# qianduoduolr/FGVC

Hardware: AMD Instinct MI355X
Metric: frames/sec + ms/corr-volume, 480p 8-frame clip, 1/2/4/8 MI355X (higher is better)
Workload: dtype f16 + fp6 (e2m3) MFMA operands, f32 accumulate; top-k near-ties re-scored in f64 from f32 features

## Files before the change

### fgvc_amd/csrc/refine.hip

```cpp
#include "common.hpp"

namespace fgvc {

constexpr int RF_KX = 16;
constexpr int RF_KMAX = 10;
constexpr int RF_BRUTE = 1 << 30;

struct RefineItem {
  int row, q, flags, m;
  int gid[RF_KX];
  float sc[RF_KX];
};
static_assert(sizeof(RefineItem) == 144, "RefineItem");
constexpr int RF_INLINE = 1 << 29;
constexpr int RF_SAMPLE = 1 << 28;

struct RefineParams {
  const int32_t* pair_idx;
  const float* pair_score;
  const int32_t* slot_pair;
  const int4* pairs;
  const unsigned char* q_exact;
  const unsigned char* k_exact;
  long long q_frame_bytes, k_frame_bytes;
  int q_row_bytes, k_row_bytes;
  int T, Hq, Wq, Hk, Wk, kin, kout;
  float temperature, eps;
  int weight_mode;
  int r2max, ry, rx, reach_y, reach_x;
  int32_t* idx_out;
  float* logit_out;
  float* weight_out;
  int* counters;
  RefineItem* items;
  int* scan_ids;
  int* scan_done;
  unsigned long long* scan_parts;
  int scan_cap;
};

__device__ __forceinline__ void rf_write(const RefineParams& p, int row, int q, const float (&sc)[RF_KMAX], const int (&id)[RF_KMAX]) {
  float lg[RF_KMAX], w[RF_KMAX];
#pragma unroll
  for (int j = 0; j < RF_KMAX; ++j) lg[j] = sc[j] / p.temperature;
  if (p.weight_mode == FGVC_WEIGHT_SOFTMAX) {
    float sum = 0.f;
#pragma unroll
    for (int j = 0; j < RF_KMAX; ++j) {
      w[j] = (j < p.kout) ? expf(lg[j] - lg[0]) : 0.f;
      sum += w[j];
    }
#pragma unroll
    for (int j = 0; j < RF_KMAX; ++j) w[j] = w[j] / sum;
  } else {
#pragma unroll
    for (int j = 0; j < RF_KMAX; ++j) {
      const float c = fmaxf(lg[j], 0.f);
      w[j] = c * c;
    }
  }
  const size_t o = ((size_t)row * p.Hq * p.Wq + q) * p.kout;
#pragma unroll
  for (int j = 0; j < RF_KMAX; ++j) {
    if (j < p.kout) {
      p.idx_out[o + j] = id[j] == IDX_EMPTY ? -1 : id[j];
      p.logit_out[o + j] = lg[j];
      p.weight_out[o + j] = w[j];
    }
  }
}

__global__ __launch_bounds__(256) void merge_mark_kernel(RefineParams p) {
  const int HWq = p.Hq * p.Wq, HWk = p.Hk * p.Wk;
  const int q_raw = blockIdx.x * 256 + threadIdx.x;
  const int f = blockIdx.y;
  const bool valid = q_raw < HWq;
  const int q = valid ? q_raw : HWq - 1;
  TopK<RF_KX> top;
  top.init();
  float drop_max = -INFINITY;
  float tau_max = -INFINITY;
  float tau[16];
#pragma unroll
  for (int t = 0; t < 16; ++t) tau[t] = -INFINITY;
  auto take = [&](int t, int id, float s) -> bool {
    const int gid = t * HWk + id;
    if (!top.accepts(s, gid)) {
      drop_max = fmaxf(drop_max, s);
      return false;
    }
    if (top.ix[RF_KX - 1] != IDX_EMPTY) drop_max = fmaxf(drop_max, top.v[RF_KX - 1]);
    top.insert(s, gid);
    return true;
  };
  if (p.kin == RF_KMAX) {
    unsigned long long a[RF_KX];
#pragma unroll
    for (int j = 0; j < RF_KX; ++j) a[j] = 0ull;
    unsigned long long dropk = 0ull;
    int2 ii[RF_KMAX / 2], ni[RF_KMAX / 2];
    float2 ss[RF_KMAX / 2], ns[RF_KMAX / 2];
    auto fetch = [&](int t, int2 (&I)[RF_KMAX / 2], float2 (&S)[RF_KMAX / 2]) -> int {
      const int pid = t < p.T ? p.slot_pair[f * p.T + t] : -1;
      if (pid >= 0) {
        const size_t o = ((size_t)pid * HWq + q) * RF_KMAX;
#pragma unroll
        for (int j = 0; j < RF_KMAX / 2; ++j) {
          I[j] = reinterpret_cast<const int2*>(p.pair_idx + o)[j];
          S[j] = reinterpret_cast<const float2*>(p.pair_score + o)[j];
        }
      }
      return pid;
    };
    int pid = fetch(0, ii, ss);
    for (int t = 0; t < p.T; ++t) {
      const int npid = fetch(t + 1, ni, ns);
      if (pid >= 0) {
        unsigned long long bk[RF_KMAX];
#pragma unroll
        for (int j = 0; j < RF_KMAX; ++j) {
          const int id = (j & 1) ? ii[j / 2].y : ii[j / 2].x;
          const float sv = (j & 1) ? ss[j / 2].y : ss[j / 2].x;
          bk[j] = id >= 0 ? TopK64<1>::make_key(sv, t * HWk + id) : 0ull;
        }
        if (bk[RF_KMAX - 1] != 0ull) {
          const float tv = ss[RF_KMAX / 2 - 1].y;
          tau_max = fmaxf(tau_max, tv);
#pragma unroll
          for (int u = 0; u < 16; ++u) tau[u] = u == t ? tv : tau[u];
        }
#pragma unroll
        for (int i = RF_KX - RF_KMAX; i < RF_KX; ++i) {
          const unsigned long long x = a[i], y = bk[RF_KX - 1 - i];
          const bool g = x > y;
          a[i] = g ? x : y;
          const unsigned long long lo = g ? y : x;
          dropk = lo > dropk ? lo : dropk;
        }
#pragma unroll
        for (int d = RF_KX / 2; d >= 1; d >>= 1)
#pragma unroll
          for (int i = 0; i < RF_KX; ++i)
            if ((i & d) == 0) {
              const unsigned long long x = a[i], y = a[i + d];
              const bool g = x > y;
              a[i] = g ? x : y;
              a[i + d] = g ? y : x;
            }
      }
      pid = npid;
#pragma unroll
      for (int j = 0; j < RF_KMAX / 2; ++j) { ii[j] = ni[j]; ss[j] = ns[j]; }
    }
    TopK64<RF_KX> dec;
#pragma unroll
    for (int j = 0; j < RF_KX; ++j) dec.k[j] = a[j];
#pragma unroll
    for (int j = 0; j < RF_KX; ++j) {
      top.v[j] = dec.score(j);
      top.ix[j] = a[j] == 0ull ? IDX_EMPTY : dec.index(j);
    }
    if (dropk != 0ull) {
      TopK64<1> dd;
      dd.k[0] = dropk;
      drop_max = dd.score(0);
    }
  } else {
    for (int t = 0; t < p.T; ++t) {
      const int pid = p.slot_pair[f * p.T + t];
      if (pid < 0) continue;
      const size_t o = ((size_t)pid * HWq + q) * p.kin;
      if (p.pair_idx[o + p.kin - 1] >= 0) {
        const float tv = p.pair_score[o + p.kin - 1];
        tau_max = fmaxf(tau_max, tv);
#pragma unroll
        for (int u = 0; u < 16; ++u) tau[u] = u == t ? tv : tau[u];
      }
      for (int j = 0; j < p.kin; ++j) {
        const int id = p.pair_idx[o + j];
        if (id < 0) break;
        if (!take(t, id, p.pair_score[o + j])) break;
      }
    }
  }
  const float two_eps = 2.f * p.eps;
  float t_k = -INFINITY;
#pragma unroll
  for (int j = 0; j < RF_KX; ++j)
    if (j == p.kout - 1 && top.ix[j] != IDX_EMPTY) t_k = top.v[j];
  const float thr = t_k - two_eps;
  int m = 0;
#pragma unroll
  for (int j = 0; j < RF_KX; ++j) m += (top.ix[j] != IDX_EMPTY && top.v[j] >= thr) ? 1 : 0;
  const bool brute = (drop_max > -INFINITY && drop_max >= thr) || (tau_max > -INFINITY && tau_max >= thr);
  unsigned twins = 0;
#pragma unroll
  for (int j = 0; j + 1 < RF_KX; ++j) {
    if (j + 1 < m && top.v[j] == top.v[j + 1]) {
      const int ta = top.ix[j] / HWk, tb = top.ix[j + 1] / HWk;
      if (top.ix[j] - ta * HWk == top.ix[j + 1] - tb * HWk && p.slot_pair[f * p.T + ta] == p.slot_pair[f * p.T + tb]) twins |= 1u << j;
    }
  }
  unsigned mask = 0;
#pragma unroll
  for (int j = 0; j + 1 < RF_KX; ++j) {
    const bool inside = j + 1 < m;
    if (inside && !((twins >> j) & 1u) && top.v[j] - top.v[j + 1] <= two_eps) mask |= 3u << j;
  }
#pragma unroll
  for (int j = 0; j + 1 < RF_KX; ++j)
    if (((twins >> j) & 1u) && ((mask >> j) & 3u)) mask |= 3u << j;
#pragma unroll
  for (int j = RF_KX - 2; j >= 0; --j)
    if (((twins >> j) & 1u) && ((mask >> j) & 3u)) mask |= 3u << j;
  const bool flagged = valid && (brute || mask != 0u);
  if (valid && !flagged) {
    float sc[RF_KMAX];
    int id[RF_KMAX];
#pragma unroll
    for (int j = 0; j < RF_KMAX; ++j) { sc[j] = top.v[j]; id[j] = top.ix[j]; }
    rf_write(p, f, q, sc, id);
  }
  const unsigned hsh = ((unsigned)q * 2654435761u) ^ ((unsigned)f * 0x9E3779B1u);
  const bool sampled = valid && !flagged && ((hsh >> 11) & 63u) == 0u;
  unsigned mask_all = 0;
#pragma unroll
  for (int j = 0; j < RF_KX; ++j) mask_all |= (top.ix[j] != IDX_EMPTY) ? (1u << j) : 0u;
  const bool queued = flagged || (sampled && mask_all != 0u);
  const int lane = threadIdx.x & 63;
  const unsigned long long lt = (1ull << lane) - 1ull;
  const unsigned long long bf = __ballot(queued), bb = __ballot(flagged && brute);
  if (bf == 0ull) return;
  int base_f = 0, base_b = 0;
  if (lane == __builtin_ctzll(bf)) base_f = atomicAdd(&p.counters[0], __popcll(bf));
  base_f = __shfl(base_f, __builtin_ctzll(bf));
  if (bb != 0ull) {
    if (lane == __builtin_ctzll(bb)) base_b = atomicAdd(&p.counters[1], __popcll(bb));
    base_b = __shfl(base_b, __builtin_ctzll(bb));
  }
  int n_resc = (flagged && !brute) ? __popc(mask) : 0;
#pragma unroll
  for (int mm = 32; mm >= 1; mm >>= 1) n_resc += __shfl_xor(n_resc, mm);
  if (lane == __builtin_ctzll(bf) && n_resc) atomicAdd(&p.counters[2], n_resc);
  int n_smp = (queued && !flagged) ? __popc(mask_all) : 0;
#pragma unroll
  for (int mm = 32; mm >= 1; mm >>= 1) n_smp += __shfl_xor(n_smp, mm);
  const int q_smp = __popcll(__ballot(queued && !flagged));
  if (lane == __builtin_ctzll(bf) && n_smp) {
    atomicAdd(&p.counters[6], n_smp);
    atomicAdd(&p.counters[7], q_smp);
  }
  if (!queued) return;
  const int slot = base_f + __popcll(bf & lt);
  int flags = flagged ? (int)mask : (RF_SAMPLE | (int)mask_all);
  if (!flagged) m = __popc(mask_all);
  if (brute) {
    const int b = base_b + __popcll(bb & lt);
    unsigned open = 0;
#pragma unroll
    for (int t = 0; t < 16; ++t) open |= (tau[t] > -INFINITY && tau[t] >= thr) ? (1u << t) : 0u;
    if (drop_max > -INFINITY && drop_max >= thr) open = 0xffffu;
    flags = RF_BRUTE | (int)open;
    if (b < p.scan_cap) p.scan_ids[b] = slot;
    else { flags |= RF_INLINE; atomicAdd(&p.counters[3], 1); }
  }
  RefineItem* it = p.items + slot;
  it->row = f; it->q = q; it->flags = flags; it->m = m;
#pragma unroll
  for (int j = 0; j < RF_KX; ++j) { it->gid[j] = top.ix[j]; it->sc[j] = top.v[j]; }
}

__device__ __forceinline__ int rf_mine(int lane) { return ((lane >> 5) & 1) * 4 + ((lane >> 4) & 1) * 2 + ((lane >> 3) & 1); }
__device__ __forceinline__ void rf_load8(const unsigned char* const (&krow)[8], int lane, f32x4 (&b)[8]) {
#pragma unroll
  for (int v = 0; v < 8; ++v) b[v] = *reinterpret_cast<const f32x4*>(krow[v] + 16 * lane);
}
__device__ __forceinline__ double rf_reduce8(const f32x4& a, const f32x4 (&b)[8], int lane) {
  double p[8];
#pragma unroll
  for (int v = 0; v < 8; ++v) {
    double s = (double)a.x * (double)b[v].x;
    s = fma((double)a.y, (double)b[v].y, s);
    s = fma((double)a.z, (double)b[v].z, s);
    s = fma((double)a.w, (double)b[v].w, s);
    p[v] = s;
  }
  const bool h5 = (lane & 32) != 0, h4 = (lane & 16) != 0, h3 = (lane & 8) != 0;
  double q4[4], q2[2];
#pragma unroll
  for (int i = 0; i < 4; ++i) q4[i] = (h5 ? p[i + 4] : p[i]) + __shfl_xor(h5 ? p[i] : p[i + 4], 32);
#pragma unroll
  for (int i = 0; i < 2; ++i) q2[i] = (h4 ? q4[i + 2] : q4[i]) + __shfl_xor(h4 ? q4[i] : q4[i + 2], 16);
  double c = (h3 ? q2[1] : q2[0]) + __shfl_xor(h3 ? q2[0] : q2[1], 8);
  c += __shfl_xor(c, 4);
  c += __shfl_xor(c, 2);
  c += __shfl_xor(c, 1);
  return c;
}
__device__ __forceinline__ double rf_dot8(const f32x4& a, const unsigned char* const (&krow)[8], int lane) {
  f32x4 b[8];
  rf_load8(krow, lane, b);
  return rf_reduce8(a, b, lane);
}

__device__ __forceinline__ void refine_item_wave(const RefineParams& p, const RefineItem* I, int lane, float& wave_err) {
  const int HWk = p.Hk * p.Wk;
  {
    const int row = __builtin_amdgcn_readfirstlane(I->row), q = __builtin_amdgcn_readfirstlane(I->q);
    const int flags = __builtin_amdgcn_readfirstlane(I->flags);
    if ((flags & RF_BRUTE) && !(flags & RF_INLINE)) return;
    int m = __builtin_amdgcn_readfirstlane(I->m);
    int gid = I->gid[lane & 15];
    float sc = I->sc[lane & 15];
    int qf = 0;
    for (int t = 0; t < p.T; ++t) {
      const int pid = p.slot_pair[row * p.T + t];
      if (pid >= 0) { qf = p.pairs[pid].x; break; }
    }
    const f32x4 qv = *reinterpret_cast<const f32x4*>(p.q_exact + (size_t)qf * p.q_frame_bytes + (size_t)q * p.q_row_bytes + 16 * lane);
    if (!(flags & RF_BRUTE)) {
      float err = 0.f;
      const unsigned char* qrow = p.q_exact + (size_t)qf * p.q_frame_bytes + (size_t)q * p.q_row_bytes;
#pragma unroll
      for (int half = 0; half < 2; ++half) {
        if (!((flags >> (8 * half)) & 255)) continue;
        const unsigned char* kr[8];
#pragma unroll
        for (int v = 0; v < 8; ++v) {
          const int e = 8 * half + v;
          kr[v] = qrow;
          if ((flags >> e) & 1) {
            const int g = __builtin_amdgcn_readlane(gid, e);
            const int t = g / HWk, pix = g - t * HWk;
            const int kf = p.pairs[p.slot_pair[row * p.T + t]].y;
            kr[v] = p.k_exact + (size_t)kf * p.k_frame_bytes + (size_t)pix * p.k_row_bytes;
          }
        }
        const float sv = (float)rf_dot8(qv, kr, lane);
#pragma unroll
        for (int v = 0; v < 8; ++v) {
          const int e = 8 * half + v;
          const int src = ((v >> 2) & 1) * 32 + ((v >> 1) & 1) * 16 + (v & 1) * 8;
          const float got = __builtin_bit_cast(float, __builtin_amdgcn_readlane(__builtin_bit_cast(int, sv), src));
          if (((flags >> e) & 1) && (lane & 15) == e) {
            err = fmaxf(err, fabsf(got - sc));
            sc = got;
          }
        }
      }
      wave_err = fmaxf(wave_err, err);
    } else {
      TopK<RF_KMAX> ex;
      ex.init();
      const int qy = q / p.Wq, qx = q - qy * p.Wq;
      for (int t = 0; t < p.T; ++t) {
        const int pid = p.slot_pair[row * p.T + t];
        if (pid < 0) continue;
        const int4 pr = p.pairs[pid];
        const bool masked = (pr.z & FGVC_PAIR_MASKED) != 0;
        const int y0 = masked ? imax(0, qy - imin(p.reach_y, qy)) : 0, y1 = masked ? imin(p.Hk - 1, qy + imin(p.reach_y, p.Hk)) : p.Hk - 1;
        const int x0 = masked ? imax(0, qx - imin(p.reach_x, qx)) : 0, x1 = masked ? imin(p.Wk - 1, qx + imin(p.reach_x, p.Wk)) : p.Wk - 1;
        const unsigned char* kb = p.k_exact + (size_t)pr.y * p.k_frame_bytes;
        for (int y = y0; y <= y1; ++y)
          for (int x = x0; x <= x1; ++x) {
            if (masked) {
              const int dy = y - qy, dx = x - qx, ady = dy < 0 ? -dy : dy, adx = dx < 0 ? -dx : dx;
              const long long d2 = (long long)dy * dy + (long long)dx * dx;
              if (!(d2 <= p.r2max && ady <= p.ry && adx <= p.rx)) continue;
            }
            const int pix = y * p.Wk + x;
            const unsigned char* r1 = kb + (size_t)pix * p.k_row_bytes;
            const unsigned char* kr[8] = {r1, r1, r1, r1, r1, r1, r1, r1};
            const float s = (float)rf_dot8(qv, kr, lane);
            const int g = t * HWk + pix;
            if (ex.accepts(s, g)) ex.insert(s, g);
          }
      }
      gid = IDX_EMPTY; sc = -INFINITY; m = 0;
#pragma unroll
      for (int j = 0; j < RF_KMAX; ++j) {
        if ((lane & 15) == j) { gid = ex.ix[j]; sc = ex.v[j]; }
        m += ex.ix[j] != IDX_EMPTY ? 1 : 0;
      }
    }
    const int i = lane & 15;
    int rank = 0;
#pragma unroll
    for (int j = 0; j < RF_KX; ++j) {
      const float sj = __builtin_bit_cast(float, __builtin_amdgcn_readlane(__builtin_bit_cast(int, sc), j));
      const int gj = __builtin_amdgcn_readlane(gid, j);
      rank += (j < m && (sj > sc || (sj == sc && gj < gid))) ? 1 : 0;
    }
    float osc[RF_KMAX];
    int oid[RF_KMAX];
#pragma unroll
    for (int r = 0; r < RF_KMAX; ++r) {
      const unsigned long long b = __ballot(lane < 16 && i < m && rank == r);
      if (b) {
        const int src = __builtin_amdgcn_readfirstlane(__builtin_ctzll(b));
        osc[r] = __builtin_bit_cast(float, __builtin_amdgcn_readlane(__builtin_bit_cast(int, sc), src));
        oid[r] = __builtin_amdgcn_readlane(gid, src);
      } else {
        osc[r] = -INFINITY;
        oid[r] = IDX_EMPTY;
      }
    }
    if (lane == 0) rf_write(p, row, q, osc, oid);
  }
}


__global__ __launch_bounds__(256) void refine_kernel(RefineParams p) {
  const int lane = threadIdx.x & 63, sub = lane & 15, g0 = lane & 48;
  const int wave = __builtin_amdgcn_readfirstlane((int)((blockIdx.x * 256 + threadIdx.x) >> 6));
  const int n_waves = (int)gridDim.x * 4;
  const int n_items = __builtin_amdgcn_readfirstlane(p.counters[0]);
  const int HWk = p.Hk * p.Wk;
  float wave_err = 0.f, wave_err_s = 0.f;
  for (int base = 4 * wave; base < n_items; base += 4 * n_waves) {
    const int it = base + (lane >> 4);
    const bool active = it < n_items;
    const RefineItem* I = p.items + (active ? it : base);
    const int row = I->row, q = I->q, flags = I->flags, m = I->m;
    int gid = I->gid[sub];
    float sc = I->sc[sub];
    const bool mine = active && !(flags & RF_BRUTE);
    const unsigned mask = mine ? ((unsigned)flags & 0xffffu) : 0u;
    const bool ent = mine && gid != IDX_EMPTY && sub < m;
    const int t_ = ent ? gid / HWk : 0, pix = ent ? gid - t_ * HWk : 0;
    const int pid = ent ? p.slot_pair[row * p.T + t_] : -1;
    const int4 pr = pid >= 0 ? p.pairs[pid] : int4{0, 0, 0, 0};
    const unsigned char* my_row = p.k_exact + (size_t)pr.y * p.k_frame_bytes + (size_t)pix * p.k_row_bytes;
    const int qf = __shfl(pr.x, g0);
    const unsigned char* qrow = p.q_exact + (size_t)qf * p.q_frame_bytes + (size_t)(mine ? q : 0) * p.q_row_bytes + 64 * sub;
    f32x4 qv[4];
    if (mine) {
#pragma unroll
      for (int j = 0; j < 4; ++j) qv[j] = *reinterpret_cast<const f32x4*>(qrow + 16 * j);
    } else {
#pragma unroll
      for (int j = 0; j < 4; ++j) qv[j] = f32x4{0.f, 0.f, 0.f, 0.f};
    }
    float err = 0.f;
    unsigned um = mask;
    um |= __shfl_xor(um, 16);
    um |= __shfl_xor(um, 32);
    um = (unsigned)__builtin_amdgcn_readfirstlane((int)um);
    while (um) {
      int ev[4];
      bool nd[4];
      f32x4 kv[4][4];
#pragma unroll
      for (int b4 = 0; b4 < 4; ++b4) {
        ev[b4] = um ? __builtin_ctz(um) : -1;
        if (um) um &= um - 1;
        nd[b4] = ev[b4] >= 0 && ((mask >> ev[b4]) & 1u);
        const unsigned long long ra = __shfl((unsigned long long)(size_t)my_row, g0 + (ev[b4] >= 0 ? ev[b4] : 0));
        const unsigned char* kr = nd[b4] ? reinterpret_cast<const unsigned char*>((size_t)ra) + 64 * sub : qrow;
#pragma unroll
        for (int j = 0; j < 4; ++j) kv[b4][j] = *reinterpret_cast<const f32x4*>(kr + 16 * j);
      }
#pragma unroll
      for (int b4 = 0; b4 < 4; ++b4) {
        if (ev[b4] < 0) continue;
        double sacc = 0.0;
#pragma unroll
        for (int j = 0; j < 4; ++j) {
          sacc = fma((double)qv[j].x, (double)kv[b4][j].x, sacc);
          sacc = fma((double)qv[j].y, (double)kv[b4][j].y, sacc);
          sacc = fma((double)qv[j].z, (double)kv[b4][j].z, sacc);
          sacc = fma((double)qv[j].w, (double)kv[b4][j].w, sacc);
        }
#pragma unroll
        for (int mm = 8; mm >= 1; mm >>= 1) sacc += __shfl_xor(sacc, mm);
        if (nd[b4] && sub == ev[b4]) {
          const float got = (float)sacc;
          err = fmaxf(err, fabsf(got - sc));
          sc = got;
        }
      }
    }
    const bool smp = mine && (flags & RF_SAMPLE) != 0;
    wave_err_s = fmaxf(wave_err_s, smp ? err : 0.f);
    wave_err = fmaxf(wave_err, smp ? 0.f : err);
    int rank = 0;
#pragma unroll
    for (int j = 0; j < RF_KX; ++j) {
      const float sj = __shfl(sc, g0 + j);
      const int gj = __shfl(gid, g0 + j);
      rank += (j < m && (sj > sc || (sj == sc && gj < gid))) ? 1 : 0;
    }
    const bool inwin = mine && !smp && sub < m;
    float osc[RF_KMAX];
    int oid[RF_KMAX];
#pragma unroll
    for (int r = 0; r < RF_KMAX; ++r) {
      const unsigned long long bal = __ballot(inwin && rank == r);
      const unsigned grp = (unsigned)(bal >> g0) & 0xffffu;
      const int src = g0 + (grp ? __builtin_ctz(grp) : 0);
      const float v = __shfl(sc, src);
      const int gi = __shfl(gid, src);
      osc[r] = grp ? v : -INFINITY;
      oid[r] = grp ? gi : IDX_EMPTY;
    }
    if (mine && !smp && sub == 0) rf_write(p, row, q, osc, oid);
  }
#pragma unroll
  for (int mm = 32; mm >= 1; mm >>= 1) {
    wave_err = fmaxf(wave_err, __shfl_xor(wave_err, mm));
    wave_err_s = fmaxf(wave_err_s, __shfl_xor(wave_err_s, mm));
  }
  if (lane == 0 && wave_err > 0.f) atomicMax(&p.counters[4], __builtin_bit_cast(int, wave_err));
  if (lane == 0 && wave_err_s > 0.f) atomicMax(&p.counters[5], __builtin_bit_cast(int, wave_err_s));
}

__global__ __launch_bounds__(256) void refine_inline_kernel(RefineParams p) {
  if (p.counters[3] == 0) return;
  const int lane = threadIdx.x & 63;
  const int wave = __builtin_amdgcn_readfirstlane((int)((blockIdx.x * 256 + threadIdx.x) >> 6));
  const int n_waves = (int)gridDim.x * 4;
  const int n_items = __builtin_amdgcn_readfirstlane(p.counters[0]);
  float wave_err = 0.f;
  for (int it = wave; it < n_items; it += n_waves) {
    const int flags = __builtin_amdgcn_readfirstlane(p.items[it].flags);
    if ((flags & RF_BRUTE) && (flags & RF_INLINE)) refine_item_wave(p, p.items + it, lane, wave_err);
  }
}

constexpr int RF_SCAN_WAVES = 8;
constexpr int RF_SCAN_PARTS = 4;

__global__ __launch_bounds__(RF_SCAN_WAVES * 64) void refine_scan_kernel(RefineParams p) {
  __shared__ unsigned long long wk[RF_SCAN_WAVES][8 * RF_KMAX];
  __shared__ unsigned long long wl[RF_SCAN_WAVES][RF_KMAX];
  __shared__ unsigned long long pl[RF_KMAX];
  __shared__ unsigned long long fk[RF_SCAN_PARTS * RF_KMAX], fl[RF_KMAX];
  __shared__ int s_last;
  const int lane = threadIdx.x & 63;
  const int wave = __builtin_amdgcn_readfirstlane((int)(threadIdx.x >> 6));
  const int n_scan = imin(p.counters[1], p.scan_cap);
  const int HWk = p.Hk * p.Wk;
  const int mine_v = rf_mine(lane);
  constexpr int NWI = RF_SCAN_WAVES * RF_SCAN_PARTS;
  for (int u = blockIdx.x; u < n_scan * RF_SCAN_PARTS; u += gridDim.x) {
    const int b = u / RF_SCAN_PARTS, part = u - b * RF_SCAN_PARTS;
    const int wi = part * RF_SCAN_WAVES + wave;
    const RefineItem* I = p.items + p.scan_ids[b];
    const int row = __builtin_amdgcn_readfirstlane(I->row), q = __builtin_amdgcn_readfirstlane(I->q);
    int qf = 0;
    for (int t = 0; t < p.T; ++t) {
      const int pid = p.slot_pair[row * p.T + t];
      if (pid >= 0) { qf = p.pairs[pid].x; break; }
    }
    const f32x4 qv = *reinterpret_cast<const f32x4*>(p.q_exact + (size_t)qf * p.q_frame_bytes + (size_t)q * p.q_row_bytes + 16 * lane);
    const int qy = q / p.Wq, qx = q - qy * p.Wq;
    TopK<RF_KMAX> loc;
    loc.init();
    const unsigned open = (unsigned)__builtin_amdgcn_readfirstlane(I->flags) & 0xffffu;
    const int m_in = __builtin_amdgcn_readfirstlane(I->m);
    int pass = 0;
    if (wi == NWI - 1) {
      const int gid = I->gid[lane & 15];
#pragma unroll
      for (int half = 0; half < 2; ++half) {
        const unsigned char* kr[8];
        bool any = false;
        int my_g = IDX_EMPTY;
#pragma unroll
        for (int v = 0; v < 8; ++v) {
          const int e = 8 * half + v;
          const int g = __builtin_amdgcn_readlane(gid, e);
          kr[v] = p.q_exact + (size_t)qf * p.q_frame_bytes + (size_t)q * p.q_row_bytes;
          if (e < m_in && g != IDX_EMPTY) {
            const int t = g / HWk, pix = g - t * HWk;
            if (!((open >> t) & 1u)) {
              kr[v] = p.k_exact + (size_t)p.pairs[p.slot_pair[row * p.T + t]].y * p.k_frame_bytes + (size_t)pix * p.k_row_bytes;
              any = true;
              if (v == mine_v) my_g = g;
            }
          }
        }
        if (any) {
          const float sc = (float)rf_dot8(qv, kr, lane);
          if (my_g != IDX_EMPTY && (lane & 7) == 0 && loc.accepts(sc, my_g)) loc.insert(sc, my_g);
        }
      }
    }
    for (int t = 0; t < p.T; ++t) {
      const int pid = p.slot_pair[row * p.T + t];
      if (pid < 0 || !((open >> t) & 1u)) continue;
      bool twin_done = false;
      for (int t2 = 0; t2 < t; ++t2) twin_done = twin_done || (((open >> t2) & 1u) && p.slot_pair[row * p.T + t2] == pid);
      if (twin_done) continue;
      const int4 pr = p.pairs[pid];
      const bool masked = (pr.z & FGVC_PAIR_MASKED) != 0;
      const int y0 = masked ? imax(0, qy - imin(p.reach_y, qy)) : 0, y1 = masked ? imin(p.Hk - 1, qy + imin(p.reach_y, p.Hk)) : p.Hk - 1;
      const int x0 = masked ? imax(0, qx - imin(p.reach_x, qx)) : 0, x1 = masked ? imin(p.Wk - 1, qx + imin(p.reach_x, p.Wk)) : p.Wk - 1;
      const int nbx = x1 - x0 + 1, nbox = (y1 - y0 + 1) * nbx, npass = (nbox + 7) / 8;
      const unsigned char* kb = p.k_exact + (size_t)pr.y * p.k_frame_bytes;
      const int first = (wi - pass % NWI + NWI) % NWI;
      auto rows_of = [&](int i, const unsigned char* (&kr)[8], int& my_pix, bool& my_ok) {
        my_pix = 0; my_ok = false;
#pragma unroll
        for (int v = 0; v < 8; ++v) {
          const int c = imin(8 * i + v, nbox - 1);
          const int yy = c / nbx;
          const int y = y0 + yy, x = x0 + (c - yy * nbx);
          bool ok = 8 * i + v < nbox;
          if (masked) {
            const int dy = y - qy, dx = x - qx, ady = dy < 0 ? -dy : dy, adx = dx < 0 ? -dx : dx;
            ok = ok && ((long long)dy * dy + (long long)dx * dx <= p.r2max && ady <= p.ry && adx <= p.rx);
          }
          const int pix = y * p.Wk + x;
          kr[v] = kb + (size_t)pix * p.k_row_bytes;
          if (v == mine_v) { my_pix = pix; my_ok = ok; }
        }
      };
      f32x4 cur[8], nxt[8];
      int pix_c = 0, pix_n = 0;
      bool ok_c = false, ok_n = false;
      if (first < npass) {
        const unsigned char* kr[8];
        rows_of(first, kr, pix_c, ok_c);
        rf_load8(kr, lane, cur);
      }
      for (int i = first; i < npass; i += NWI) {
        const bool more = i + NWI < npass;
        if (more) {
          const unsigned char* kr[8];
          rows_of(i + NWI, kr, pix_n, ok_n);
          rf_load8(kr, lane, nxt);
        }
        const float sc = (float)rf_reduce8(qv, cur, lane);
        for (int t2 = t; t2 < p.T; ++t2) {
          if (t2 > t && !(((open >> t2) & 1u) && p.slot_pair[row * p.T + t2] == pid)) continue;
          const int g = t2 * HWk + pix_c;
          if (ok_c && (lane & 7) == 0 && loc.accepts(sc, g)) loc.insert(sc, g);
        }
        if (more) {
#pragma unroll
          for (int v = 0; v < 8; ++v) cur[v] = nxt[v];
          pix_c = pix_n; ok_c = ok_n;
        }
      }
      pass += npass;
    }
    __syncthreads();
    if ((lane & 7) == 0) {
#pragma unroll
      for (int j = 0; j < RF_KMAX; ++j)
        wk[wave][(lane >> 3) * RF_KMAX + j] = loc.ix[j] == IDX_EMPTY ? 0ull : TopK64<1>::make_key(loc.v[j], loc.ix[j]);
    }
    if (lane < RF_KMAX) wl[wave][lane] = 0ull;
    if (threadIdx.x < RF_KMAX) pl[threadIdx.x] = 0ull;
    {
      asm volatile("s_waitcnt lgkmcnt(0)" ::: "memory");
      const unsigned long long ka = wk[wave][lane], kb2 = lane < 8 * RF_KMAX - 64 ? wk[wave][64 + lane] : 0ull;
      int ra = 0, rb = 0;
      for (int j = 0; j < 8 * RF_KMAX; ++j) {
        const unsigned long long kj = wk[wave][j];
        ra += kj > ka ? 1 : 0;
        rb += kj > kb2 ? 1 : 0;
      }
      if (ka != 0ull && ra < RF_KMAX) wl[wave][ra] = ka;
      if (kb2 != 0ull && rb < RF_KMAX) wl[wave][rb] = kb2;
    }
    __syncthreads();
    if (threadIdx.x < RF_SCAN_WAVES * RF_KMAX) {
      const unsigned long long ka = wl[threadIdx.x / RF_KMAX][threadIdx.x % RF_KMAX];
      int ra = 0;
      for (int j = 0; j < RF_SCAN_WAVES * RF_KMAX; ++j) ra += wl[j / RF_KMAX][j % RF_KMAX] > ka ? 1 : 0;
      if (ka != 0ull && ra < RF_KMAX) pl[ra] = ka;
    }
    __syncthreads();
    if (wave == 0) {
      unsigned long long* dst = p.scan_parts + ((size_t)b * RF_SCAN_PARTS + part) * RF_KMAX;
      if (lane < RF_KMAX) dst[lane] = pl[lane];
      __threadfence();
      if (lane == 0) s_last = atomicAdd(&p.scan_done[b], 1) == RF_SCAN_PARTS - 1;
    }
    __syncthreads();
    if (s_last && wave == 0) {
      __threadfence();
      const unsigned long long* src = p.scan_parts + (size_t)b * RF_SCAN_PARTS * RF_KMAX;
      constexpr int NE = RF_SCAN_PARTS * RF_KMAX;
      static_assert(NE <= 128, "two keys per lane");
      const unsigned long long ka = lane < NE ? __hip_atomic_load(src + lane, __ATOMIC_RELAXED, __HIP_MEMORY_SCOPE_AGENT) : 0ull;
      const unsigned long long kb2 = lane + 64 < NE ? __hip_atomic_load(src + lane + 64, __ATOMIC_RELAXED, __HIP_MEMORY_SCOPE_AGENT) : 0ull;
      if (lane < NE) fk[lane] = ka;
      if (lane + 64 < NE) fk[lane + 64] = kb2;
      if (lane < RF_KMAX) fl[lane] = 0ull;
      asm volatile("s_waitcnt lgkmcnt(0)" ::: "memory");
      int ra = 0, rb = 0;
      for (int j = 0; j < NE; ++j) {
        const unsigned long long kj = fk[j];
        ra += kj > ka ? 1 : 0;
        rb += kj > kb2 ? 1 : 0;
      }
      if (ka != 0ull && ra < RF_KMAX) fl[ra] = ka;
      if (kb2 != 0ull && rb < RF_KMAX) fl[rb] = kb2;
      asm volatile("s_waitcnt lgkmcnt(0)" ::: "memory");
      if (lane == 0) {
        float osc[RF_KMAX];
        int oid[RF_KMAX];
        TopK64<RF_KMAX> dec;
#pragma unroll
        for (int j = 0; j < RF_KMAX; ++j) dec.k[j] = fl[j];
#pragma unroll
        for (int j = 0; j < RF_KMAX; ++j) {
          osc[j] = dec.score(j);
          oid[j] = dec.k[j] == 0ull ? IDX_EMPTY : dec.index(j);
        }
        rf_write(p, row, q, osc, oid);
      }
    }
  }
}

size_t merge_refine_scan_cap(int n_out, int HWq) { return (size_t)imax(4096, (int)(((long long)n_out * HWq + 31) / 32)); }

int merge_refine_launch(const RefineParams& p_in, int n_out, void* workspace, hipStream_t s) {
  RefineParams p = p_in;
  p.scan_cap = (int)merge_refine_scan_cap(n_out, p.Hq * p.Wq);
  const size_t cap4 = (((size_t)p.scan_cap * 4 + 15) / 16) * 16;
  p.counters = reinterpret_cast<int*>(workspace);
  unsigned char* w = reinterpret_cast<unsigned char*>(workspace) + 64;
  p.scan_done = reinterpret_cast<int*>(w);
  w += cap4;
  p.scan_ids = reinterpret_cast<int*>(w);
  w += cap4;
  p.scan_parts = reinterpret_cast<unsigned long long*>(w);
  w += (size_t)p.scan_cap * RF_SCAN_PARTS * RF_KMAX * 8;
  p.items = reinterpret_cast<RefineItem*>(w);
  if (hipMemsetAsync(workspace, 0, 64 + cap4, s) != hipSuccess) {
    set_error("fgvc_merge_refine_topk_f32: hipMemsetAsync failed");
    return FGVC_ERR_LAUNCH;
  }
  dim3 grid(cdiv(p.Hq * p.Wq, 256), n_out);
  merge_mark_kernel<<<grid, 256, 0, s>>>(p);
  FGVC_CHECK_LAUNCH("fgvc_merge_refine_topk_f32 (merge)");
  refine_kernel<<<1024, 256, 0, s>>>(p);
  FGVC_CHECK_LAUNCH("fgvc_merge_refine_topk_f32 (refine)");
  refine_inline_kernel<<<1024, 256, 0, s>>>(p);
  FGVC_CHECK_LAUNCH("fgvc_merge_refine_topk_f32 (inline)");
  refine_scan_kernel<<<1024, RF_SCAN_WAVES * 64, 0, s>>>(p);
  FGVC_CHECK_LAUNCH("fgvc_merge_refine_topk_f32 (scan)");
  return FGVC_OK;
}

}

using namespace fgvc;

extern "C" {

size_t fgvc_merge_refine_workspace_bytes(int n_out, int HWq) {
  if (n_out < 0 || HWq < 0) return 0;
  const size_t cap = fgvc::merge_refine_scan_cap(n_out, HWq);
  return 64 + 2 * (((cap * 4 + 15) / 16) * 16) + cap * fgvc::RF_SCAN_PARTS * fgvc::RF_KMAX * 8 + (size_t)n_out * HWq * sizeof(RefineItem);
}

int fgvc_merge_refine_topk_f32(const int32_t* pair_idx, const float* pair_score, const int32_t* slot_pair, const int32_t* pairs,
                               const void* q_exact, int64_t q_frame_bytes, int q_row_bytes, const void* k_exact, int64_t k_frame_bytes,
                               int k_row_bytes, int n_out, int T, int Hq, int Wq, int Hk, int Wk, int C, int topk, float temperature,
                               int weight_mode, float eps, int r2max, int ry, int rx, int32_t* idx_out, float* logit_out,
                               float* weight_out, void* workspace, void* stream) {
  const char* what = "fgvc_merge_refine_topk_f32";
  FGVC_REQUIRE(pair_idx && pair_score && slot_pair && pairs && q_exact && k_exact && idx_out && logit_out && weight_out && workspace,
               FGVC_ERR_INVALID_ARG, "%s: null pointer", what);
  FGVC_REQUIRE(C == 256, FGVC_ERR_UNSUPPORTED, "%s: C=%d unsupported (256 only)", what, C);
  FGVC_REQUIRE(topk >= 1 && topk <= RF_KMAX, FGVC_ERR_UNSUPPORTED, "%s: topk=%d outside 1..%d", what, topk, RF_KMAX);
  FGVC_REQUIRE(T <= 16, FGVC_ERR_UNSUPPORTED, "%s: T=%d key slots (at most 16)", what, T);
  FGVC_REQUIRE(n_out >= 0 && n_out <= 65535 && T >= 1 && Hq > 0 && Wq > 0 && Hk > 0 && Wk > 0, FGVC_ERR_INVALID_ARG, "%s: bad shape", what);
  FGVC_REQUIRE((long long)Hq * Wq < (1ll << 30) && (long long)Hk * Wk * T < (1ll << 31), FGVC_ERR_UNSUPPORTED, "%s: grid too large", what);
  FGVC_REQUIRE(q_row_bytes >= 1024 && k_row_bytes >= 1024 && q_row_bytes % 16 == 0 && k_row_bytes % 16 == 0 &&
                   (reinterpret_cast<uintptr_t>(q_exact) & 15u) == 0 && (reinterpret_cast<uintptr_t>(k_exact) & 15u) == 0 &&
                   q_frame_bytes % 16 == 0 && k_frame_bytes % 16 == 0,
               FGVC_ERR_INVALID_ARG, "%s: the exact rows are 256 f32 = 1024 bytes each, 16-byte aligned", what);
  FGVC_REQUIRE((reinterpret_cast<uintptr_t>(pairs) & 15u) == 0 && (reinterpret_cast<uintptr_t>(workspace) & 15u) == 0, FGVC_ERR_INVALID_ARG,
               "%s: pairs / workspace must be 16-byte aligned", what);
  FGVC_REQUIRE(temperature > 0.f && eps >= 0.f && eps < 1.f, FGVC_ERR_INVALID_ARG, "%s: bad temperature / eps", what);
  FGVC_REQUIRE(weight_mode == FGVC_WEIGHT_SOFTMAX || weight_mode == FGVC_WEIGHT_COSINE, FGVC_ERR_INVALID_ARG, "%s: bad weight mode", what);
  FGVC_REQUIRE(r2max >= 0 && ry >= 0 && rx >= 0, FGVC_ERR_INVALID_ARG, "%s: negative mask parameter", what);
  const bool any_limit = r2max < FGVC_NO_LIMIT || ry < FGVC_NO_LIMIT || rx < FGVC_NO_LIMIT;
  FGVC_REQUIRE(!any_limit || (Hq == Hk && Wq == Wk), FGVC_ERR_INVALID_ARG, "%s: a spatial mask needs equal query/key grids", what);
  if (n_out == 0) return FGVC_OK;
  RefineParams p;
  p.pair_idx = pair_idx; p.pair_score = pair_score; p.slot_pair = slot_pair; p.pairs = reinterpret_cast<const int4*>(pairs);
  p.q_exact = static_cast<const unsigned char*>(q_exact); p.k_exact = static_cast<const unsigned char*>(k_exact);
  p.q_frame_bytes = q_frame_bytes; p.k_frame_bytes = k_frame_bytes; p.q_row_bytes = q_row_bytes; p.k_row_bytes = k_row_bytes;
  p.T = T; p.Hq = Hq; p.Wq = Wq; p.Hk = Hk; p.Wk = Wk; p.kin = topk; p.kout = topk;
  p.temperature = temperature; p.eps = eps; p.weight_mode = weight_mode;
  p.r2max = r2max; p.ry = ry; p.rx = rx;
  int rr = 0;
  while (rr < 46340 && (long long)(rr + 1) * (rr + 1) <= (long long)r2max) ++rr;
  p.reach_y = imin(ry, rr); p.reach_x = imin(rx, rr);
  p.idx_out = idx_out; p.logit_out = logit_out; p.weight_out = weight_out;
  p.counters = nullptr; p.items = nullptr; p.scan_ids = nullptr; p.scan_done = nullptr; p.scan_parts = nullptr; p.scan_cap = 0;
  return merge_refine_launch(p, n_out, workspace, (hipStream_t)stream);
}

}
```

Baseline: 2008.

## Aggregate refine queue atomics per workgroup and fold inline pass into refine kernel

In the merge/mark kernel, per-wave atomics on the queue counters are replaced by a workgroup-level reduction in shared memory. Slot and brute counters are then claimed with one packed 64-bit atomic per workgroup, and each wave's base is derived from prefix sums. The separate inline-refine kernel is merged into the tail of refine_kernel, which also reduces its error maxima per workgroup and launches with a smaller fixed grid. This removes one kernel launch and cuts global atomic contention, at the cost of two extra __syncthreads in the mark kernel and inline work now being serialized after the main refine loop in each wave.

```diff
diff --git a/fgvc_amd/csrc/refine.hip b/fgvc_amd/csrc/refine.hip
--- a/fgvc_amd/csrc/refine.hip
+++ b/fgvc_amd/csrc/refine.hip
@@ -228,27 +228,42 @@
   for (int j = 0; j < RF_KX; ++j) mask_all |= (top.ix[j] != IDX_EMPTY) ? (1u << j) : 0u;
   const bool queued = flagged || (sampled && mask_all != 0u);
   const int lane = threadIdx.x & 63;
+  __shared__ int wg_n[4][5];
+  __shared__ int wg_base[2];
+  const int wv = threadIdx.x >> 6;
   const unsigned long long lt = (1ull << lane) - 1ull;
   const unsigned long long bf = __ballot(queued), bb = __ballot(flagged && brute);
-  if (bf == 0ull) return;
-  int base_f = 0, base_b = 0;
-  if (lane == __builtin_ctzll(bf)) base_f = atomicAdd(&p.counters[0], __popcll(bf));
-  base_f = __shfl(base_f, __builtin_ctzll(bf));
-  if (bb != 0ull) {
-    if (lane == __builtin_ctzll(bb)) base_b = atomicAdd(&p.counters[1], __popcll(bb));
-    base_b = __shfl(base_b, __builtin_ctzll(bb));
-  }
   int n_resc = (flagged && !brute) ? __popc(mask) : 0;
 #pragma unroll
   for (int mm = 32; mm >= 1; mm >>= 1) n_resc += __shfl_xor(n_resc, mm);
-  if (lane == __builtin_ctzll(bf) && n_resc) atomicAdd(&p.counters[2], n_resc);
   int n_smp = (queued && !flagged) ? __popc(mask_all) : 0;
 #pragma unroll
   for (int mm = 32; mm >= 1; mm >>= 1) n_smp += __shfl_xor(n_smp, mm);
   const int q_smp = __popcll(__ballot(queued && !flagged));
-  if (lane == __builtin_ctzll(bf) && n_smp) {
-    atomicAdd(&p.counters[6], n_smp);
-    atomicAdd(&p.counters[7], q_smp);
+  if (lane == 0) {
+    wg_n[wv][0] = __popcll(bf); wg_n[wv][1] = __popcll(bb); wg_n[wv][2] = n_resc; wg_n[wv][3] = n_smp; wg_n[wv][4] = q_smp;
+  }
+  __syncthreads();
+  if (threadIdx.x == 0) {
+    int sum[5];
+#pragma unroll
+    for (int c = 0; c < 5; ++c) sum[c] = wg_n[0][c] + wg_n[1][c] + wg_n[2][c] + wg_n[3][c];
+    unsigned long long old = 0ull;
+    if (sum[0] | sum[1])
+      old = atomicAdd(reinterpret_cast<unsigned long long*>(p.counters), (unsigned long long)(unsigned)sum[0] | ((unsigned long long)(unsigned)sum[1] << 32));
+    wg_base[0] = (int)(unsigned)old;
+    wg_base[1] = (int)(unsigned)(old >> 32);
+    if (sum[2]) atomicAdd(&p.counters[2], sum[2]);
+    if (sum[3] | sum[4])
+      atomicAdd(reinterpret_cast<unsigned long long*>(p.counters + 6), (unsigned long long)(unsigned)sum[3] | ((unsigned long long)(unsigned)sum[4] << 32));
+  }
+  __syncthreads();
+  if (bf == 0ull) return;
+  int base_f = wg_base[0], base_b = wg_base[1];
+#pragma unroll
+  for (int w2 = 0; w2 < 3; ++w2) {
+    base_f += w2 < wv ? wg_n[w2][0] : 0;
+    base_b += w2 < wv ? wg_n[w2][1] : 0;
   }
   if (!queued) return;
   const int slot = base_f + __popcll(bf & lt);
@@ -410,11 +425,14 @@
 }
 
 
+constexpr int RF_REFINE_WGS = 768;
+
 __global__ __launch_bounds__(256) void refine_kernel(RefineParams p) {
   const int lane = threadIdx.x & 63, sub = lane & 15, g0 = lane & 48;
   const int wave = __builtin_amdgcn_readfirstlane((int)((blockIdx.x * 256 + threadIdx.x) >> 6));
   const int n_waves = (int)gridDim.x * 4;
   const int n_items = __builtin_amdgcn_readfirstlane(p.counters[0]);
+  const int n_beyond = __builtin_amdgcn_readfirstlane(p.counters[3]);
   const int HWk = p.Hk * p.Wk;
   float wave_err = 0.f, wave_err_s = 0.f;
   for (int base = 4 * wave; base < n_items; base += 4 * n_waves) {
@@ -510,20 +528,18 @@
     wave_err = fmaxf(wave_err, __shfl_xor(wave_err, mm));
     wave_err_s = fmaxf(wave_err_s, __shfl_xor(wave_err_s, mm));
   }
-  if (lane == 0 && wave_err > 0.f) atomicMax(&p.counters[4], __builtin_bit_cast(int, wave_err));
-  if (lane == 0 && wave_err_s > 0.f) atomicMax(&p.counters[5], __builtin_bit_cast(int, wave_err_s));
-}
-
-__global__ __launch_bounds__(256) void refine_inline_kernel(RefineParams p) {
-  if (p.counters[3] == 0) return;
-  const int lane = threadIdx.x & 63;
-  const int wave = __builtin_amdgcn_readfirstlane((int)((blockIdx.x * 256 + threadIdx.x) >> 6));
-  const int n_waves = (int)gridDim.x * 4;
-  const int n_items = __builtin_amdgcn_readfirstlane(p.counters[0]);
-  float wave_err = 0.f;
+  __shared__ float wg_err[4][2];
+  if (lane == 0) { wg_err[threadIdx.x >> 6][0] = wave_err; wg_err[threadIdx.x >> 6][1] = wave_err_s; }
+  __syncthreads();
+  if (threadIdx.x < 2) {
+    const float e = fmaxf(fmaxf(wg_err[0][threadIdx.x], wg_err[1][threadIdx.x]), fmaxf(wg_err[2][threadIdx.x], wg_err[3][threadIdx.x]));
+    if (e > 0.f) atomicMax(&p.counters[4 + threadIdx.x], __builtin_bit_cast(int, e));
+  }
+  if (n_beyond == 0) return;
+  float unused_err = 0.f;
   for (int it = wave; it < n_items; it += n_waves) {
     const int flags = __builtin_amdgcn_readfirstlane(p.items[it].flags);
-    if ((flags & RF_BRUTE) && (flags & RF_INLINE)) refine_item_wave(p, p.items + it, lane, wave_err);
+    if ((flags & RF_BRUTE) && (flags & RF_INLINE)) refine_item_wave(p, p.items + it, lane, unused_err);
   }
 }
 
@@ -739,10 +755,8 @@
   dim3 grid(cdiv(p.Hq * p.Wq, 256), n_out);
   merge_mark_kernel<<<grid, 256, 0, s>>>(p);
   FGVC_CHECK_LAUNCH("fgvc_merge_refine_topk_f32 (merge)");
-  refine_kernel<<<1024, 256, 0, s>>>(p);
+  refine_kernel<<<RF_REFINE_WGS, 256, 0, s>>>(p);
   FGVC_CHECK_LAUNCH("fgvc_merge_refine_topk_f32 (refine)");
-  refine_inline_kernel<<<1024, 256, 0, s>>>(p);
-  FGVC_CHECK_LAUNCH("fgvc_merge_refine_topk_f32 (inline)");
   refine_scan_kernel<<<1024, RF_SCAN_WAVES * 64, 0, s>>>(p);
   FGVC_CHECK_LAUNCH("fgvc_merge_refine_topk_f32 (scan)");
   return FGVC_OK;
```

New measurement: 2046 (median of 6 runs). 1.02x the previous value.
